# marcinmiklitz/pywindow

Hardware: AMD Instinct MI355X
Metric: trajectory frames/sec full_analysis (pore+windows), CC3 1k-frame (higher is better)
Workload: dtype f64

## Files before the change

### pywindow_amd/csrc/pw_unit.hpp

```cpp
#pragma once
#include "../../include/pywindow_amd.h"
#include "pw_lbfgsb.hpp"
#include "pw_math.hpp"
#include "pw_team.hpp"
#include <string.h>

#if defined(PW_PROFILE) && defined(__HIPCC__)
__shared__ unsigned long long pw_prof_lds[32];
#define PW_PROF_BASE(ws) ((unsigned long long*)pw_prof_lds)
#endif
#if defined(PW_PROFILE) && defined(__HIP_DEVICE_COMPILE__)
#define PW_T0(var) long long var = wall_clock64()
#if defined(PW_ZPROF) && defined(PW_LB_FINE)
#define PW_T1(ws, slot, var) do { (void)var; } while (0)
#elif defined(PW_BARRIER_PROF)
#define PW_T1(ws, slot, var) do { (void)var; if (T::lane() == 0) { unsigned long long w_ = 0; \
        for (int k_ = 0; k_ < T::NWAVES; ++k_) w_ += atomicExch(&pw_bar_acc[k_], 0ull); \
        atomicAdd(&pw_prof_lds[slot], w_); } } while (0)
#else
#define PW_T1(ws, slot, var) do { if (T::lane() == 0) atomicAdd(&pw_prof_lds[slot], (unsigned long long)(wall_clock64() - var)); } while (0)
#endif
#else
#define PW_T0(var) do {} while (0)
#define PW_T1(ws, slot, var) do {} while (0)
// ... 1131 lines not shown
    return ::asin(x);
#else
    return __builtin_asin(x);
#endif
}
PW_HD inline double cone_atan2(double y, double x) {
#if defined(__HIP_DEVICE_COMPILE__)
    return ::atan2(y, x);
#else
    return __builtin_atan2(y, x);
#endif
}
PW_HD inline ConeLattice cone_lattice_window(double rx, double ry, double rz, double rr, double thr, double R) {
    ConeLattice L;
    L.c = 0.0; L.w = 1.0; L.j = -1; L.first = 0; L.plen = 1;
    const double len = pw_sqrt(rr);
    const double ct = thr / (R * len) - 1e-12;
    if (!(ct > 0.0)) return L;
    const double sa = pw_sqrt(pw_max(1.0 - ct * ct, 0.0));
    const double rho = pw_sqrt(rx * rx + ry * ry) / len;
    if (!(rho > sa * (1.0 + 1e-6) + 1e-9)) return L;
    const double delta = cone_asin(sa / rho) * (1.0 + 1e-9) + 1e-9;
    const double w = delta / ONE_PI;
    int j = 0;
    while (j + 1 < ConeLatticeTable::N && pw_abs(CONE_LATTICE_TABLE.s[j]) > w) ++j;
    if (j + 1 >= ConeLatticeTable::N) return L;
    double c = (cone_atan2(ry, rx) - delta) / TWO_PI;
    c -= __builtin_floor(c);
    L.c = c < 1.0 ? c : 0.0;
    L.w = w;
    L.j = (short)j;
    return L;
}
struct ConeLatticeWalk {
    double t, w, a, b;
    int k, A, B;
    PW_HD void enter(const ConeLattice& L, int k0, int kend) {
        const int j = L.j, pos = j & 1 ? j + 1 : j, neg = j & 1 ? j : j + 1;
        A = CONE_LATTICE_TABLE.q[pos]; a = CONE_LATTICE_TABLE.s[pos];
        B = CONE_LATTICE_TABLE.q[neg]; b = -CONE_LATTICE_TABLE.s[neg];
        w = L.w;
        k = k0;
        t = (double)k0 * CONE_LATTICE_G - L.c;
        t -= __builtin_floor(t);
        while (k <= kend && !(t < w)) {
            ++k;
            t += CONE_LATTICE_G;
            if (t >= 1.0) t -= 1.0;
        }
    }
    PW_HD void next() {
        if (t + a < w) { k += A; t += a; }
        else if (t - b >= 0.0) { k += B; t -= b; }
        else { k += A + B; t = (t + a) - b; }
    }
};
PW_HD inline ConeLattice* take_cone_lattice(ScratchArena& a, int n) {
#ifdef PW_NO_CONE_LATTICE
    (void)a; (void)n;
    return nullptr;
#else
    return (ConeLattice*)a.take((size_t)(n + 1) * sizeof(ConeLattice));
#endif
}
PW_HD inline __attribute__((always_inline)) int cone_of_atom(double rx, double ry, double rz, double vr, double cn, const Sphere& sp,
                                                            bool narrow, ConeBand* out, ConeLattice* lat_out) {
    const int P = sp.P;
    ConeBand b;
    ConeLattice L;
    L.c = 0.0; L.w = 1.0; L.j = -1; L.first = 0; L.plen = 1;
    int cnt = 0;
    const double rr = sq3(rx, ry, rz);
    const double a2 = rr - pw_fma(rr, 1e-12, (vr * vr) * (1.0 + 1e-12));
    b.klo = 0; b.khi = -P;
    b.thr = -PW_INF;
    if (a2 > 0.0) {
        const double amin = pw_sqrt(a2) * (1.0 - 1e-9);
        b.thr = amin * sp.R * (1.0 - 1e-9);
        if (amin > cn + 1e-6) {
            const double len = pw_sqrt(rr);
            const double zd = rz / len, c = amin / len;
            const double s_ = pw_sqrt(pw_max(1.0 - c * c, 0.0)) * (1.0 + 1e-9) + 1e-9;
            const double rho = pw_sqrt(pw_max(1.0 - zd * zd, 0.0));
            const double zhi = zd >= c ? 1.0 : pw_min(1.0, zd * c + rho * s_ + 1e-9);
            const double zlo = zd <= -c ? -1.0 : pw_max(-1.0, zd * c - rho * s_ - 1e-9);
            const double kh = (zlo - sp.start) / sp.step, kl = (zhi - sp.start) / sp.step;
            b.klo = (int)pw_max(kl - 2.0, 0.0);
            b.khi = (int)pw_min(kh + 3.0, (double)(P - 1));
            if (narrow) {
                L = cone_lattice_window(rx, ry, rz, rr, b.thr, sp.R);
                if (L.j >= 0) {
                    cnt = cone_pieces(b.khi - b.klo + 1, L.w, &L.plen);
                    b.klo = ~b.klo;
                }
            }
        }
    }
    *out = b;
    *lat_out = L;
    return cnt;
}
template <class T, bool FAR, class GETP>
PW_HD inline __attribute__((always_inline)) bool team_ray_tests(const Frame& F, int n, const double* cen, const Sphere& sp,
                                                               GETP getp, ConeBand* bands, unsigned* pairs, int cap,
                                                               PW_LDS int* counts, unsigned char* flag,
                                                               unsigned char hit_value, double* far,
                                                               ConeLattice* lat = nullptr) {
    const int P = sp.P;
    const int seg = cap / T::NWAVES;
    if (P >= 65536 || n >= 65536 || seg < 64) return false;
    const double c0 = cen[0], c1 = cen[1], c2 = cen[2];
    const double cn = norm3(c0, c1, c2);
    int running = 0;
    for (int base = 0; base < n; base += T::SIZE) {
        const int i = base + T::tid();
        ConeBand b;
        ConeLattice L;
        int cnt = 0;
        if (i < n) {
            cnt = cone_of_atom(F.x[i] - c0, F.y[i] - c1, F.z[i] - c2, F.vdw[i], cn, sp, lat != nullptr, &b, &L);
            bands[i] = b;
        }
        if (lat != nullptr) {
            const int inc = T::incl_scan_i(cnt);
            if (T::lane() == T::WSIZE - 1) counts[T::wave()] = inc;
            T::sync();
            int at = running + inc - cnt;
#pragma unroll
            for (int w = 0; w < T::NWAVES; ++w) { const int cw = counts[w]; if (w < T::wave()) at += cw; running += cw; }
            if (i < n) { L.first = at; lat[i] = L; }
            T::sync();
        }
    }
    if (lat != nullptr && T::tid() == 0) lat[n].first = running;
    T::sync();
    int mine = 0;
    unsigned* my = pairs + (size_t)T::wave() * seg;
    auto enumerate = [&](auto bands_, auto lat_, auto my_) __attribute__((always_inline)) {
        for (int g0 = T::wave() * T::WSIZE; g0 < running; g0 += T::SIZE) {
            const int g = g0 + T::lane();
            ConeLatticeWalk wk;
            wk.k = 1;
            int kend = 0, i = 0;
            double rx = 0.0, ry = 0.0, rz = 0.0, thr = 0.0;
            if (g < running) {
                int lo = 0, hi = n - 1;
                while (lo < hi) {
                    const int mid = (lo + hi) >> 1;
                    if (lat_[mid + 1].first > g) hi = mid; else lo = mid + 1;
                }
                i = lo;
                const ConeBand b = bands_[i];
                const ConeLattice L = lat_[i];
                const int k0 = ~b.klo + (g - L.first) * (int)L.plen;
                kend = k0 + (int)L.plen - 1 < b.khi ? k0 + (int)L.plen - 1 : b.khi;
                rx = F.x[i] - c0; ry = F.y[i] - c1; rz = F.z[i] - c2;
                thr = b.thr;
                wk.enter(L, k0, kend);
            }
            while (T::wave_any(wk.k <= kend)) {
                const bool act = wk.k <= kend;
                const int k = wk.k;
                bool f = false;
                if (act) {
                    double px, py, pz;
                    getp(k, &px, &py, &pz);
                    const double dot = pw_fma(pz, rz, pw_fma(px, rx, py * ry));
                    f = dot >= thr;
                    wk.next();
                }
                const unsigned long long bal = T::ballot(f);
                const int pos = mine + __builtin_popcountll(bal & ((1ull << T::lane()) - 1ull));
                if (f && pos < seg) my_[pos] = ((unsigned)k << 16) | (unsigned)i;
                mine += __builtin_popcountll(bal);
            }
        }
    };
    if (lat != nullptr) {
        if (PW_IS_LDS(bands) && PW_IS_LDS(lat) && PW_IS_LDS(my)) enumerate(PW_AS_LDS(bands), PW_AS_LDS(lat), PW_AS_LDS(my));
        else enumerate(bands, lat, my);
    }
    for (int i = T::wave(); i < n; i += T::NWAVES) {
        const ConeBand b = bands[i];
        if (b.klo < 0) continue;
        const bool two_sided = b.khi < 0;
        const int khi = two_sided ? -b.khi - 1 : b.khi;
        const double rx = F.x[i] - c0, ry = F.y[i] - c1, rz = F.z[i] - c2;
        int off = getp.first(b.klo + T::lane());
        for (int kb = b.klo; kb <= khi; kb += T::WSIZE, off += GETP::STEP64) {
            const int k = kb + T::lane();
            bool f = false;
            if (k <= khi) {
                double px, py, pz;
                if (T::WSIZE == 64) getp.at(off, &px, &py, &pz);
                else getp(k, &px, &py, &pz);
                const double dot = pw_fma(pz, rz, pw_fma(px, rx, py * ry));
                f = two_sided ? pw_abs(dot) >= b.thr : dot >= b.thr;
            }
            const unsigned long long bal = T::ballot(f);
            const int pos = mine + __builtin_popcountll(bal & ((1ull << T::lane()) - 1ull));
            if (f && pos < seg) my[pos] = ((unsigned)k << 16) | (unsigned)i;
            mine += __builtin_popcountll(bal);
        }
    }
    if (T::lane() == 0) counts[T::wave()] = mine;
    T::sync();
    int cum[T::NWAVES + 1];
    cum[0] = 0;
    bool fits = true;
#pragma unroll
    for (int w = 0; w < T::NWAVES; ++w) { const int cw = counts[w]; fits = fits && cw <= seg; cum[w + 1] = cum[w] + cw; }
    T::sync();
    if (!fits) return false;
    for (int g = T::tid(); g < cum[T::NWAVES]; g += T::SIZE) {
        int w = 0, first = 0;
#pragma unroll
        for (int q = 1; q < T::NWAVES; ++q)
            if (g >= cum[q]) { w = q; first = cum[q]; }
        const unsigned pr = pairs[(size_t)w * seg + (g - first)];
        const int k = (int)(pr >> 16), i = (int)(pr & 0xffffu);
        double dx, dy, dz;
        getp(k, &dx, &dy, &dz);
        const double nrm = norm3(dx, dy, dz);
        const double ux = dx / nrm, uy = dy / nrm, uz = dz / nrm;
        const double rx = F.x[i] - c0, ry = F.y[i] - c1, rz = F.z[i] - c2;
        const double along = pw_fma(rz, uz, pw_fma(rx, ux, ry * uy));
        const double sq = sq3(rx, ry, rz);
        const double perp = pw_sqrt(sq - along * along);
        const double radicand = F.vdw[i] * F.vdw[i] - perp * perp;
        if (radicand > 0.0) {
            const double half = pw_sqrt(radicand);
            const double tin = along - half, tout = along + half;
            const double ix = c0 + tin * ux, iy = c1 + tin * uy, iz = c2 + tin * uz;
            const double ox = c0 + tout * ux, oy = c1 + tout * uy, oz = c2 + tout * uz;
            const double nin = norm3(ix, iy, iz), nout = norm3(ox, oy, oz);
            if (nin < nout) {
                flag[k] = hit_value;
                if (FAR) team_store_max_pos(&far[k], nout);
            }
        }
    }
    T::sync();
    return true;
}

PW_HD inline double np_floordiv(double a, double b) {
    double mod = __builtin_fmod(a, b);
    double div = (a - mod) / b;
    if (mod != 0.0) {
        if ((b < 0.0) != (mod < 0.0)) div -= 1.0;
    }
    double fl;
    if (div != 0.0) {
        fl = __builtin_floor(div);
        if (div - fl > 0.5) fl += 1.0;
    } else {
        fl = 0.0;
    }
    return fl;
}

PW_NOINLINE PW_HD inline bool path_scan_thread(const Frame& F, int n, double vx, double vy, double vz,
                                   double inc, double m0, double* out_2gap, int* out_pos, double* out_chunk,
                                   int* n_eval, const lint* cand = nullptr, const lint* coff = nullptr) {
    double nrm = norm3(vx, vy, vz);
    int chunks = (int)np_floordiv(nrm, inc);
    double cx = vx / (double)chunks, cy = vy / (double)chunks, cz = vz / (double)chunks;
    double best = PW_INF;
    int pos = 0;
    bool ok = true;
    int k0 = 0;
    if (chunks >= 1) {
        if (!(m0 > 0.0)) ok = false;
        best = m0;
        k0 = 1;
    }
    auto tile = [&](auto np_) __attribute__((always_inline)) {
        constexpr int NP = decltype(np_)::value;
        double qx[NP], qy[NP], qz[NP], m[NP];
#pragma unroll
        for (int p = 0; p < NP; ++p) {
            int k = k0 + p <= chunks ? k0 + p : chunks;
            qx[p] = cx * (double)k; qy[p] = cy * (double)k; qz[p] = cz * (double)k;
        }
        points_gap_values<NP>(F, n, qx, qy, qz, m, cand, coff);
#pragma unroll
        for (int p = 0; p < NP; ++p) {
            if (k0 + p <= chunks && ok) {
                if (!(m[p] > 0.0)) ok = false;
                else if (m[p] < best) { best = m[p]; pos = k0 + p; }
            }
        }
        k0 += NP;
    };
    while (k0 <= chunks && ok) {
        if (chunks - k0 + 1 <= 5) tile(std::integral_constant<int, 5>());
        else tile(std::integral_constant<int, 6>());
    }
    if (n_eval) *n_eval += chunks + 1;
    if (!ok) return false;
    *out_2gap = best * 2.0;
    *out_pos = pos;
    out_chunk[0] = cx; out_chunk[1] = cy; out_chunk[2] = cz;
    return true;
}

template <class T>
PW_HD inline bool wave_path_candidates(const Frame& F, int n, bool have, double vx, double vy, double vz, double inc,
                                       double m0, lint* cand, lint* coff) {
    const auto& C = *F.cls;
    if (C.k == 0 || !(m0 > 0.0)) return false;
    double uz_lo = PW_INF, uz_hi = -PW_INF, t1 = PW_INF;
    bool odd = false;
    if (have) {
        const double nrm = norm3(vx, vy, vz);
        odd = !(nrm >= inc * (1.0 + 1e-9)) || !(nrm < PW_INF) || !(inc > 0.0);
        if (!odd) uz_lo = uz_hi = vz / nrm;
    }
    if (T::wave_any(odd)) return false;
    double z1 = T::wave_min(uz_lo) - 1e-9, z2 = -T::wave_min(-uz_hi) + 1e-9;
    t1 = inc * (1.0 - 1e-9);
    if (!(z1 <= z2)) return false;
    z1 = pw_max(z1, -1.0); z2 = pw_min(z2, 1.0);
    const double s1 = pw_sqrt(pw_max(1.0 - z1 * z1, 0.0)), s2 = pw_sqrt(pw_max(1.0 - z2 * z2, 0.0));
    const double m0p = m0 * (1.0 + 1e-9) + 1e-9;
    const int mycut = T::lane() <= C.k ? C.off[T::lane() <= PW_KCLS ? T::lane() : PW_KCLS] : n;
    int mycount = 0, cnt = 0;
    for (int base = 0; base < n; base += T::WSIZE) {
        const int i = base + T::lane();
        bool keep = false;
        if (i < n) {
            const double xx = F.xx[i], z = F.z[i], r = F.vdw[i];
            const double rho = pw_sqrt(xx);
            const double zd = rho > 0.0 ? z / rho : 0.0;
            const double sd = pw_sqrt(pw_max(1.0 - zd * zd, 0.0));
            double c1 = 1.0;
            if (zd > z2) c1 = sd * s2 + zd * z2;
            else if (zd < z1) c1 = sd * s1 + zd * z1;
            c1 = pw_min(1.0, pw_max(0.0, c1 + 1e-9));
            const double ts = rho * c1;
            const double low = ts >= t1 ? xx * (1.0 - c1 * c1) : (xx + t1 * t1) - 2.0 * t1 * ts;
            const double lim = (r + m0p) * (r + m0p);
            keep = !(low * (1.0 - 1e-9) - 1e-9 > lim * (1.0 + 1e-9));
        }
        const unsigned long long bal = T::ballot(keep);
        const int pos = cnt + __builtin_popcountll(bal & ((1ull << T::lane()) - 1ull));
        if (keep) cand[pos] = i;
        if (T::WSIZE > 1) {
            int w = mycut - base;
            w = w < 0 ? 0 : (w > 64 ? 64 : w);
            mycount += __builtin_popcountll(bal & (w >= 64 ? ~0ull : ((1ull << w) - 1ull)));
        }
        cnt += __builtin_popcountll(bal);
    }
    if (T::WSIZE > 1) {
        if (T::lane() <= C.k) coff[T::lane()] = mycount;
    } else {
        int c = 0;
        for (int g = 0; g <= C.k; ++g) {
            while (c < cnt && cand[c] < C.off[g]) ++c;
            coff[g] = c;
        }
    }
    T::wave_sync();
    return true;
}

PW_HD inline size_t template_groups_bytes(int n) {
    const size_t npad = (size_t)((n + 1) & ~1);
    return ((sizeof(ClassInfo) + 7) & ~(size_t)7) + npad * 4 * 2 + npad * 8 + 8;
}
PW_HD inline double molecular_weight_sum(const double* mass, int n) {
    double tot = 0.0;
    for (int s0 = 0; s0 < n; s0 += 8192) {
        double part = np_sum_lean(mass + s0, n - s0 < 8192 ? n - s0 : 8192);
        tot = s0 == 0 ? part : tot + part;
    }
    return tot;
}
inline void template_groups_build(const double* vdw, const double* mass, int n, unsigned char* blob) {
    const size_t npad = (size_t)((n + 1) & ~1);
    ClassInfo* cls = (ClassInfo*)blob;
    int* inv = (int*)(blob + ((sizeof(ClassInfo) + 7) & ~(size_t)7));
    int* perm = inv + npad;
    double* vs = (double*)(perm + npad);
    memset(blob, 0, template_groups_bytes(n));
    int ngrp = 0;
    for (int i = 0; i < n; ++i) {
        int key = i;
        for (int j = 0; j < i; ++j)
            if (vdw[j] == vdw[i]) { key = j; break; }
        perm[i] = key;
        if (key == i) ++ngrp;
    }
    if (ngrp > PW_KCLS) {
        cls->k = 0; cls->off[0] = 0;
        for (int i = 0; i < n; ++i) inv[i] = i;
    } else {
        cls->k = ngrp;
        for (int i = 0; i < n; ++i) {
            const int key = perm[i];
            int pos = 0, cid = 0;
            for (int j = 0; j < n; ++j) {
                const int kj = perm[j];
                pos += (kj < key) || (kj == key && j < i);
                cid += (kj == j) && (j < key);
            }
            inv[i] = pos;
            if (key == i) { cls->vdw[cid] = vdw[i]; cls->off[cid] = pos; }
        }
        cls->off[ngrp] = n;
    }
    for (int i = 0; i < n; ++i) { vs[inv[i]] = vdw[i]; }
    for (int i = 0; i < n; ++i) perm[inv[i]] = i;
    vs[npad] = molecular_weight_sum(mass, n);
}

template <class T>
PW_HD inline void load_unit(UnitShared& sh, int n, const double* xyz, const double* vdw,
                            const double* mass, const unsigned char* tmpl = nullptr) {
    auto& v = *sh.v;
    if (tmpl) {
        const size_t npad = (size_t)((n + 1) & ~1);
        const ClassInfo* tc = (const ClassInfo*)tmpl;
        const int* t_inv = (const int*)(tmpl + ((sizeof(ClassInfo) + 7) & ~(size_t)7));
        const int* t_perm = t_inv + npad;
        const double* t_vs = (const double*)(t_perm + npad);
        for (int i = T::tid(); i < n; i += T::SIZE) {
            const int pos = t_inv[i];
            const double x = xyz[3 * i], y = xyz[3 * i + 1], z = xyz[3 * i + 2];
            sh.A.x[pos] = x; sh.A.y[pos] = y; sh.A.z[pos] = z;
            sh.A.xx[pos] = sq3(x, y, z);
            sh.inv[i] = pos;
            sh.perm[i] = t_perm[i];
            sh.vdw[i] = t_vs[i];
            sh.mass[i] = mass[i];
        }
        if (T::tid() == 0) {
            v.n_eval = 0; v.status = 0;
            v.mw = t_vs[npad]; v.mw_given = 1;
            v.cls.k = tc->k;
            for (int g = 0; g <= PW_KCLS; ++g) v.cls.off[g] = tc->off[g];
            for (int g = 0; g < PW_KCLS; ++g) v.cls.vdw[g] = tc->vdw[g];
        }
        T::sync();
        return;
    }
    for (int i = T::tid(); i < n; i += T::SIZE) {
        double r = vdw[i];
        sh.vdw[i] = r;
        sh.mass[i] = mass[i];
    }
    if (T::tid() == 0) { v.n_eval = 0; v.status = 0; v.cls.k = 0; v.mw_given = 0; }
    T::sync();
    for (int i = T::tid(); i < n; i += T::SIZE) {
        double r = sh.vdw[i];
        int key = i;
        for (int j = 0; j < i; ++j)
            if (sh.vdw[j] == r) { key = j; break; }
        sh.perm[i] = key;
    }
    T::sync();
    for (int i = T::tid(); i < n; i += T::SIZE) {
        int key = sh.perm[i];
        int pos = 0, cid = 0;
        for (int j = 0; j < n; ++j) {
            int kj = sh.perm[j];
            pos += (kj < key) || (kj == key && j < i);
            cid += (kj == j) && (j < key);
        }
        sh.inv[i] = pos;
        if (key == i) {
            if (cid < PW_KCLS) { v.cls.vdw[cid] = sh.vdw[i]; v.cls.off[cid] = pos; }
            team_atomic_max(&v.cls.k, cid + 1);
        }
    }
    T::sync();
    const int ngrp = v.cls.k;
    T::sync();
    if (ngrp > PW_KCLS) {
        for (int i = T::tid(); i < n; i += T::SIZE) sh.inv[i] = i;
        if (T::tid() == 0) { v.cls.k = 0; v.cls.off[0] = 0; }
    } else if (T::tid() == 0) {
        v.cls.off[ngrp] = n;
    }
    T::sync();
    for (int i = T::tid(); i < n; i += T::SIZE) {
        int pos = sh.inv[i];
        double x = xyz[3 * i], y = xyz[3 * i + 1], z = xyz[3 * i + 2];
        sh.A.x[pos] = x; sh.A.y[pos] = y; sh.A.z[pos] = z;
        sh.A.xx[pos] = sq3(x, y, z);
        sh.vdw[pos] = vdw[i];
        sh.perm[pos] = i;
    }
    T::sync();
}

template <int B, class F>
PW_HD inline double seq_sum_blocks(int n, F term) {
    double s = term(0);
    int i = 1;
    for (; i + B <= n; i += B) {
        double v[B];
#pragma unroll
        for (int j = 0; j < B; ++j) v[j] = term(i + j);
#pragma unroll
        for (int j = 0; j < B; ++j) s = s + v[j];
    }
    for (; i < n; ++i) s = s + term(i);
    return s;
}
template <class F>
PW_HD inline double seq_sum_blocked(int n, F term) { return seq_sum_blocks<8>(n, term); }

template <class T>
PW_HD inline ldouble* seq_sum_columns(const UnitShared& sh, int n) {
    const size_t np = (size_t)((n + 1) & ~1);
    if (T::SIZE < 64 || sh.scratch_bytes < 3 * np * 8) return nullptr;
    return (ldouble*)sh.scratch;
}
template <class T, class FIN>
PW_HD inline void seq_sum_columns_add(const ldouble* cols, int n, FIN fin) {
    const size_t np = (size_t)((n + 1) & ~1);
    if (T::tid() < 3) {
        const ldouble* a = cols + (size_t)T::tid() * np;
        fin(T::tid(), seq_sum_blocks<16>(n, [&](int i) { return a[i]; }));
    }
}

template <class T>
PW_HD inline void make_shifted(UnitShared& sh, int n, double cx, double cy, double cz) {
    ldouble* cols = seq_sum_columns<T>(sh, n);
    const size_t np = (size_t)((n + 1) & ~1);
    for (int i = T::tid(); i < n; i += T::SIZE) {
        double x = sh.A.x[i] - cx, y = sh.A.y[i] - cy, z = sh.A.z[i] - cz;
        sh.S.x[i] = x; sh.S.y[i] = y; sh.S.z[i] = z;
        sh.S.xx[i] = sq3(x, y, z);
        if (cols) { const int ci = sh.perm[i]; cols[ci] = x; cols[np + ci] = y; cols[2 * np + ci] = z; }
    }
    T::sync();
    if (cols) {
        seq_sum_columns_add<T>(cols, n, [&](int c, double s) { sh.v->centroid[c] = s / (double)n; });
        T::sync();
        return;
    }
    auto cen_comp = [&](int c) {
        const ldouble* a = c == 0 ? sh.S.x : (c == 1 ? sh.S.y : sh.S.z);
        double s = seq_sum_blocked(n, [&](int i) { return a[sh.inv[i]]; });
        sh.v->centroid[c] = s / (double)n;
    };
    if (T::SIZE >= 3) {
        if (T::tid() < 3) cen_comp(T::tid());
    } else if (T::tid() == 0) {
        cen_comp(0); cen_comp(1); cen_comp(2);
    }
    T::sync();
}

struct GramEdgeRule {
    int t0, panel, panel_wide, nfull, limlast;
    PW_HD static bool applies(int n) { return n % 8 >= 4; }
    PW_HD static int last_panel_start(int n) {
        int start = 0;
        for (;;) {
            const int rem = n - start;
            const int mi = rem >= 384 ? 192 : (rem > 192 ? 32 * ((rem / 2 + 31) / 32) : rem);
            if (start + mi >= n) return start;
            start += mi;
        }
    }
    PW_HD explicit GramEdgeRule(int n) {
        t0 = applies(n) ? 8 * (n / 8) : 0x40000000;
        panel = last_panel_start(n);
        panel_wide = 12 * (panel / 12);
        nfull = 32 * (n / 32);
        limlast = 12 * ((n - nfull) / 12);
    }
    PW_HD bool is_edge(int o) const { return (unsigned)(o - t0) < 4u; }
    PW_HD bool in_wide_kernel(int o) const {
        return o < panel ? o < panel_wide : (o & 31) < (o < nfull ? 24 : limlast);
    }
    PW_HD bool pair_uses_edge_order(int oi, int oj) const {
        return (is_edge(oi) && in_wide_kernel(oj)) || (is_edge(oj) && in_wide_kernel(oi));
    }
};
template <bool EDGE>
PW_HD inline __attribute__((always_inline)) double pw_gram_nn(double xi, double yi, double zi, double xj, double yj,
                                                              double zj, int oi, int oj, const GramEdgeRule& er) {
    if (EDGE && er.pair_uses_edge_order(oi, oj)) return pw_fma(zi, zj, xi * xj + yi * yj);
    return pw_fma(zi, zj, pw_fma(yi, yj, xi * xj));
}

#if defined(__HIP_DEVICE_COMPILE__)
template <class T, bool VALUE_ONLY, bool EDGE>
__device__ inline __attribute__((always_inline)) bool team_max_dim_few(UnitShared& sh, const Frame& F, int n,
                                                                       const GramEdgeRule& er, const double* centre) {
    auto& v = *sh.v;
    const double cx = centre ? centre[0] : 0.0, cy = centre ? centre[1] : 0.0, cz = centre ? centre[2] : 0.0;
    double smax = -PW_INF, nmax = 0.0;
    int imax = 0x7fffffff;
    for (int i = T::tid(); i < n; i += T::SIZE) {
        const double dx = F.x[i] - cx, dy = F.y[i] - cy, dz = F.z[i] - cz;
        const double si = pw_sqrt(dx * dx + dy * dy + dz * dz) + F.vdw[i];
        if (si > smax) { smax = si; imax = i; }
        nmax = pw_max(nmax, F.xx[i]);
    }
// ... 1509 lines not shown
            v.status |= PW_ST_PATH_TOO_LONG;
            out->n_points = 0; out->sphere_r = radius; out->n_windows = -1; out->n_clusters = 0; out->n_survivors = 0; out->eps = 0.0;
        }
        T::sync();
        return -1;
    }
    int P = sampling_count(radius, prm.adjust_windows);
    if (T::tid() == 0) {
        out->n_points = P;
        out->sphere_r = radius;
        out->n_windows = -1;
        out->n_clusters = 0;
        out->n_survivors = 0;
        out->eps = 0.0;
    }
    if (P > ws->p_cap || P < 10) {
        if (T::tid() == 0) v.status |= P < 10 ? PW_ST_TOO_FEW_POINTS : PW_ST_POINTS_OVERFLOW;
        T::sync();
        return -1;
    }
    Sphere sp;
    sp.init(radius, P);
    ScratchArena arena;
    arena.init(sh);
    const int Q4 = (P + 3) >> 2;
    double* pts = (double*)arena.take((size_t)Q4 * 12 * 8);
    if (!pts) pts = ws->pts;
    auto PT = [Q4](int k, int c) { return (c * 4 + (k & 3)) * Q4 + (k >> 2); };
    ScratchArena arena_pts = arena;
    team_sphere_points<T>(ws, sp, [&](int k, double x, double y, double z) { pts[PT(k, 0)] = x; pts[PT(k, 1)] = y; pts[PT(k, 2)] = z; });
    T::sync();
    if (T::wave() == 0) PW_T1(ws, 26, t_pre);
    PW_T0(t_eps);
    {
        PW_T0(t_knn);
        constexpr int NK = 4;
        const int ngroups = (P + NK - 1) / NK;
        int* s_tab = (int*)arena.take(324 * 4);
        double* s_leaf = (double*)arena.take(256 * 8);
        double* s_acc = nullptr;
        double* tile = nullptr;
        int tile_cap = 0;
        if (s_tab && s_leaf && T::SIZE > 1 && ngroups <= T::SIZE) {
            long words = (long)(arena.left / 8) - 160;
            int slots = (int)(words / (64 + 8)) - 2;
            if (slots > 64) slots = 64;
            if (slots >= 4) {
                size_t acc_words = 8 * (size_t)(slots + 2);
                if (acc_words < 128) acc_words = 128;
                s_acc = (double*)arena.take(acc_words * 8);
                tile = (double*)arena.take((size_t)slots * 64 * 8);
                tile_cap = slots * 64 - 128;
            }
        }
        const bool streamed = tile != nullptr && s_acc != nullptr && tile_cap >= 128;
        if (!streamed) {
            arena = arena_pts;
            s_tab = (int*)arena.take(324 * 4);
            s_acc = (double*)arena.take(8 * 160 * 8);
            s_leaf = (double*)arena.take(256 * 8);
            if (!s_tab || !s_acc || !s_leaf) { s_tab = ws->leaf_tab; s_acc = ws->acc8; s_leaf = ws->leaf; }
        }
        const unsigned short* nb_idx = nullptr;
        const double* nb_bound = nullptr;
        if (ws->nb_off && P >= PW_NB_PMIN && P <= PW_NB_PMAX && ws->nb_off[P] != PW_NB_NONE) {
            nb_idx = ws->nb_idx + (size_t)ws->nb_off[P] * PW_NB_K;
            nb_bound = ws->nb_bound + ws->nb_off[P];
        }
        const int W = (int)(0.118 * (double)P) + 6;
        const double zstep = pw_abs(sp.step) * radius;
        auto point_tabled = [&](auto pts_, int k, double* d10) __attribute__((always_inline)) {
            if (!nb_idx) return false;
            const double slack = (radius * radius) * (1.0 - 1e-9);
            const double px = pts_[PT(k, 0)], py = pts_[PT(k, 1)], pz = pts_[PT(k, 2)];
            const unsigned* row = (const unsigned*)(nb_idx + (size_t)k * PW_NB_K);
            unsigned w[8];
#pragma unroll
            for (int c = 0; c < 8; ++c) w[c] = row[c];
            double prev = -1.0, cd[PW_NB_K];
            bool sorted = true;
#pragma unroll
            for (int c = 0; c < PW_NB_K; ++c) {
                const int j = (int)((w[c >> 1] >> (16 * (c & 1))) & 0xffffu);
                const double qx = pts_[PT(j, 0)], qy = pts_[PT(j, 1)], qz = pts_[PT(j, 2)];
                double ax = px - qx, ay = py - qy, az = pz - qz;
                double d = ax * ax;
                d = d + ay * ay; d = d + az * az;
                sorted = sorted && d >= prev;
                prev = d;
                cd[c] = d;
                if (c < 10) d10[c] = d;
            }
            if (!sorted) {
#pragma unroll
                for (int q = 0; q < 10; ++q) d10[q] = PW_INF;
#pragma unroll
                for (int c = 0; c < PW_NB_K; ++c) {
                    double v_ = cd[c];
#pragma unroll
                    for (int q = 0; q < 10; ++q) {
                        double lo_ = __builtin_fmin(d10[q], v_);
                        v_ = __builtin_fmax(d10[q], v_);
                        d10[q] = lo_;
                    }
                }
            }
            const bool ok = d10[9] < nb_bound[k] * slack;
#pragma unroll
            for (int q = 0; q < 10; ++q) d10[q] = pw_sqrt(d10[q]);
            return ok;
        };
        auto point_dists = [&](auto pts_, int grp, int k, bool& searched, double* d10) __attribute__((always_inline)) {
            if (!searched && point_tabled(pts_, k, d10)) return;
            if (!searched) {
                knn_window_group(pts_, Q4, P, grp, W, radius, zstep, ws->knn);
                searched = true;
            }
#pragma unroll
            for (int q = 0; q < 10; ++q) d10[q] = ws->knn[(size_t)k * 10 + q];
        };
        if (!streamed) {
            auto rows_of_groups = [&](auto pts_) __attribute__((always_inline)) {
                for (int grp = T::tid(); grp < ngroups; grp += T::SIZE) {
                    bool searched = false;
                    for (int p = 0; p < NK; ++p) {
                        const int k = grp * NK + p;
                        if (k >= P) break;
                        double d10[10];
                        point_dists(pts_, grp, k, searched, d10);
                        if (!searched) {
#pragma unroll
                            for (int q = 0; q < 10; ++q) ws->knn[(size_t)k * 10 + q] = d10[q];
                        }
                    }
                }
            };
            if (PW_IS_LDS(pts)) rows_of_groups(PW_AS_LDS(pts)); else rows_of_groups(pts);
        }
        T::sync();
        if (T::wave() == 0) PW_T1(ws, 24, t_knn);
        PW_T0(t_sum);
        double sum;
        if (streamed) {
            const int n_el = P * 10;
            const int grp = T::tid();
            const int e_first = grp * NK * 10;
            bool searched = false;
            double total = 0.0;
            bool first = true;
            for (int s0 = 0; s0 < n_el; s0 += 8192) {
                const int len = n_el - s0 < 8192 ? n_el - s0 : 8192;
                np_leaf_table<T>(len, s_tab);
                int lo = 0;
                while (lo < len) {
                    int hi = len;
                    if (lo + tile_cap < len) {
                        int off, l;
                        np_descend(len, lo + tile_cap, &off, &l);
                        hi = off;
                    }
                    auto fill = [&](auto tile_, auto pts_) __attribute__((always_inline)) {
                        if (nb_idx) {
                            const int E0 = s0 + lo, E1 = s0 + hi;
                            const int k1 = (E1 - 1) / 10;
                            for (int k = E0 / 10 + T::tid(); k <= k1; k += T::SIZE) {
                                double d10[10];
                                if (!point_tabled(pts_, k, d10)) {
                                    knn_window_group(pts_, Q4, P, k / NK, W, radius, zstep, ws->knn);
#pragma unroll
                                    for (int q = 0; q < 10; ++q) d10[q] = ws->knn[(size_t)k * 10 + q];
                                }
                                const int e0 = k * 10 - s0;
#pragma unroll
                                for (int q = 0; q < 10; ++q)
                                    if (e0 + q >= lo && e0 + q < hi) tile_[e0 + q - lo] = d10[q];
                            }
                            return;
                        }
                        if (grp >= ngroups) return;
                        for (int p = 0; p < NK; ++p) {
                            const int k = grp * NK + p;
                            const int e0 = e_first + p * 10 - s0;
                            if (k >= P || e0 + 10 <= lo || e0 >= hi) continue;
                            double d10[10];
                            point_dists(pts_, grp, k, searched, d10);
#pragma unroll
                            for (int q = 0; q < 10; ++q)
                                if (e0 + q >= lo && e0 + q < hi) tile_[e0 + q - lo] = d10[q];
                        }
                    };
                    if (PW_IS_LDS(tile) && PW_IS_LDS(pts)) fill(PW_AS_LDS(tile), PW_AS_LDS(pts)); else fill(tile, pts);
                    T::sync();
                    np_leaf_phase<T>(tile, len, lo, hi, s_tab, s_acc, s_leaf, true);
                    lo = hi;
                }
                double part = np_walk_phase<T>(len, s_tab, s_acc, s_leaf);
                if (T::tid() == 0) total = first ? part : total + part;
                first = false;
                T::sync();
            }
            if (T::tid() == 0) v.red_v[15] = total;
            T::sync();
            sum = v.red_v[15];
            T::sync();
        } else {
            sum = np_sum_team<T>(ws->knn, P * 10, s_tab, s_acc, s_leaf, &v.red_v[15]);
        }
        double m = sum / (double)(P * 10);
        if (T::tid() == 0) { v.eps = m + pw_pow_np(m, 0.5); out->eps = v.eps; }
        T::sync();
        if (T::wave() == 0) PW_T1(ws, 25, t_sum);
    }
    if (T::wave() == 0) PW_T1(ws, 8, t_eps);
    PW_T0(t_smp);
    arena = arena_pts;
    double* vals = (double*)arena.take((size_t)P * 8);
    if (!vals) vals = ws->vals;
    int* surv_k = (int*)arena.take((size_t)P * 4);
    if (!surv_k) surv_k = ws->surv_k;
    int* labels = (int*)arena.take((size_t)P * 4);
    if (!labels) labels = ws->labels;
    unsigned char* flag = (unsigned char*)arena.take((size_t)P);
    if (!flag) flag = ws->flag;
    ScratchArena arena_mark = arena;
    double* tmpv = (double*)arena.take((size_t)P * 8);
    if (!tmpv) tmpv = ws->knn;
    {
        double cen[3] = {v.centroid[0], v.centroid[1], v.centroid[2]};
        bool done = false;
        {
            for (int k = T::tid(); k < P; k += T::SIZE) flag[k] = 1;
            ScratchArena a2 = arena_mark;
            ConeBand* bands = (ConeBand*)a2.take((size_t)n * sizeof(ConeBand));
            ConeLattice* lat = bands ? take_cone_lattice(a2, n) : nullptr;
            int cap = (int)(a2.left / 4);
            unsigned* pairs = (unsigned*)a2.take((size_t)cap * 4);
            if (cap < 4 * P) { pairs = (unsigned*)ws->knn; cap = 16 * ws->p_cap; }
            if (!bands && (size_t)n * sizeof(ConeBand) <= (size_t)ws->p_cap * 16) bands = (ConeBand*)(ws->knn + 8 * (size_t)ws->p_cap);
            auto run = [&](auto pts_) __attribute__((always_inline)) {
                SpiralRays<decltype(pts_)> getp{pts_, Q4};
                return team_ray_tests<T, false>(sh.S, n, cen, sp, getp, bands, pairs, cap, (PW_LDS int*)&v.red_i[0], flag, 0, nullptr, lat);
            };
            if (bands) done = PW_IS_LDS(pts) ? run(PW_AS_LDS(pts)) : run(pts);
        }
        if (done) {
        } else if (T::SIZE > 1) {
            constexpr int NR = 4;
            for (int k0 = T::tid(); k0 < P; k0 += NR * T::SIZE) {
                double dx[NR], dy[NR], dz[NR], far[NR];
                bool hit[NR];
#pragma unroll
                for (int r = 0; r < NR; ++r) {
                    int k = k0 + r * T::SIZE < P ? k0 + r * T::SIZE : k0;
                    dx[r] = pts[PT(k, 0)]; dy[r] = pts[PT(k, 1)]; dz[r] = pts[PT(k, 2)];
                }
                ray_scan_multi<NR, false>(sh.S, n, cen, dx, dy, dz, hit, far);
#pragma unroll
                for (int r = 0; r < NR; ++r) {
                    int k = k0 + r * T::SIZE;
                    if (k < P) flag[k] = hit[r] ? 0 : 1;
                }
            }
        } else {
            for (int k = T::tid(); k < P; k += T::SIZE) {
                double far;
                bool hit = ray_scan(sh.S, n, cen, pts[PT(k, 0)], pts[PT(k, 1)], pts[PT(k, 2)], &far);
                flag[k] = hit ? 0 : 1;
            }
        }
        T::sync();
        if (T::wave() == 0) {
            int m = 0;
            for (int base = 0; base < P; base += T::WSIZE) {
                int k = base + T::lane();
                bool f = k < P && flag[k] != 0;
                unsigned long long bal = T::ballot(f);
                int pos = m + __builtin_popcountll(bal & ((1ull << T::lane()) - 1ull));
                if (f) labels[pos] = k;
                m += __builtin_popcountll(bal);
            }
            if (T::lane() == 0) v.n_surv = m;
        }
        T::sync();
        int ncand = v.n_surv;
        int evals = 0;
        if (T::wave() == 0) PW_T1(ws, 30, t_smp);
        PW_T0(t_path);
        const double m_origin = wave_gap_value<T>(sh.S, n, 0.0, 0.0, 0.0);
        int whole = T::SIZE > 1 ? (ncand / T::SIZE) * T::SIZE : ncand;
        if ((ncand - whole) * 16 >= T::SIZE) whole = ncand;
        lint* cand_w = nullptr;
        lint* coff_w = nullptr;
        {
            ScratchArena a3 = arena;
            const size_t per_wave = (size_t)n + PW_KCLS + 2;
            int* c_all = (int*)a3.take((size_t)T::NWAVES * per_wave * 4);
#ifndef PW_NO_SCAN_LISTS
            if (c_all && PW_IS_LDS(c_all)) {
                cand_w = (lint*)PW_AS_LDS(c_all) + (size_t)T::wave() * per_wave;
                coff_w = cand_w + n;
            }
#endif
        }
        for (int j0 = 0; j0 < whole; j0 += T::SIZE) {
            const int j = j0 + T::tid();
            const bool have = j < whole;
            const int k = have ? labels[j] : 0;
            const double vx = pts[PT(k, 0)], vy = pts[PT(k, 1)], vz = pts[PT(k, 2)];
            const bool listed = cand_w != nullptr &&
                                wave_path_candidates<T>(sh.S, n, have, vx, vy, vz, prm.increment, m_origin, cand_w, coff_w);
            if (have) {
                double g2, chunk[3];
                int pos;
                bool ok = path_scan_thread(sh.S, n, vx, vy, vz, prm.increment, m_origin, &g2, &pos, chunk, &evals,
                                           listed ? cand_w : nullptr, listed ? coff_w : nullptr);
                flag[j] = ok ? 1 : 0;
                tmpv[j] = g2;
            }
        }
        const int left = ncand - whole;
        if (left > 0) {
            for (int j = whole + T::wave(); j < ncand; j += T::NWAVES) {
                const int k = labels[j];
                const double vx = pts[PT(k, 0)], vy = pts[PT(k, 1)], vz = pts[PT(k, 2)];
                const int chunks = (int)np_floordiv(norm3(vx, vy, vz), prm.increment);
                double g2 = 0.0;
                bool ok = true;
                bool all_at_once = false;
                if constexpr (T::WSIZE == 64) all_at_once = chunks >= 1 && chunks <= 16 && sh.S.cls->k > 0;
                if (all_at_once) {
                    if constexpr (T::WSIZE == 64) {
                        const auto& C = *sh.S.cls;
                        const Frame& F = sh.S;
                        const double cx = vx / (double)chunks, cy = vy / (double)chunks, cz = vz / (double)chunks;
                        const int sub = T::lane() & 3;
                        const int q = (T::lane() >> 2) + 1 <= chunks ? (T::lane() >> 2) + 1 : chunks;
                        const double qx = cx * (double)q, qy = cy * (double)q, qz = cz * (double)q;
                        const double pp = sq3(qx, qy, qz);
                        double gap = PW_INF;
                        for (int g = 0; g < C.k; ++g) {
                            double m2 = PW_INF;
                            const int hi = C.off[g + 1];
                            for (int i = C.off[g] + sub; i < hi; i += 4) {
                                const double x = F.x[i], y = F.y[i], z = F.z[i], xx = F.xx[i];
                                const double gg = pw_fma(z, qz, pw_fma(x, qx, y * qy));
                                m2 = __builtin_fmin(m2, pw_m2add(gg, xx));
                            }
                            m2 = __builtin_fmin(m2, T::xor_d(m2, 1));
                            m2 = __builtin_fmin(m2, T::xor_d(m2, 2));
                            const double m2p = m2 + pp;
                            const double d = pw_sqrt(m2p > 0.0 ? m2p : 0.0);
                            gap = __builtin_fmin(gap, d - C.vdw[g]);
                        }
                        double best = m_origin;
                        if (!(m_origin > 0.0)) ok = false;
                        for (int q2 = 1; q2 <= chunks && ok; ++q2) {
                            const double m = T::bcast_u(gap, 4 * (q2 - 1));
                            if (!(m > 0.0)) ok = false;
                            else if (m < best) best = m;
                        }
                        g2 = best * 2.0;
                    }
                } else if (chunks >= 1) {
                    const double cx = vx / (double)chunks, cy = vy / (double)chunks, cz = vz / (double)chunks;
                    double best = m_origin;
                    if (!(m_origin > 0.0)) ok = false;
                    for (int q = 1; q <= chunks && ok; ++q) {
                        const double m = wave_gap_value<T>(sh.S, n, cx * (double)q, cy * (double)q, cz * (double)q);
                        if (!(m > 0.0)) ok = false;
                        else if (m < best) best = m;
                    }
                    g2 = best * 2.0;
                } else {
                    double chunk[3];
                    int pos;
                    ok = path_scan_thread(sh.S, n, vx, vy, vz, prm.increment, m_origin, &g2, &pos, chunk, &evals);
                }
                if (T::lane() == 0) { flag[j] = ok ? 1 : 0; tmpv[j] = g2; }
            }
        }
        T::sync();
        if (T::wave() == 0) PW_T1(ws, 31, t_path);
        if (T::wave() == 0) {
            int m = 0;
            for (int base = 0; base < ncand; base += T::WSIZE) {
                int j = base + T::lane();
                bool f = j < ncand && flag[j] != 0;
                unsigned long long bal = T::ballot(f);
                int pos = m + __builtin_popcountll(bal & ((1ull << T::lane()) - 1ull));
                if (f) { surv_k[pos] = labels[j]; vals[pos] = tmpv[j]; }
                m += __builtin_popcountll(bal);
            }
            if (T::lane() == 0) { v.n_surv = m; out->n_survivors = m; }
        }
        T::sync();
        (void)evals;
    }
    if (T::wave() == 0) PW_T1(ws, 9, t_smp);
    int ns = v.n_surv;
    if (ns == 0) {
        if (T::tid() == 0) out->n_windows = -1;
        T::sync();
        return -1;
    }
    PW_T0(t_db);
    arena = arena_mark;
    {
        const int label = team_dbscan<T>(sh.bits[0], sh.bits[1], sh.bits[2], arena, ws, pts, PT, surv_k, ns, v.eps, labels);
        if (label < 0) {
            if (T::tid() == 0) v.status |= PW_ST_POINTS_OVERFLOW;
            T::sync();
            return -1;
        }
        if (T::tid() == 0) {
            v.n_clusters = label;
            out->n_clusters = label;
        }
        if (label > PW_W_MAX) {
            wa.vec = ws->xw; wa.d = ws->xw + 3 * (size_t)ws->p_cap; wa.c = ws->xw + 4 * (size_t)ws->p_cap; wa.ok = ws->xw_ok;
        }
        for (int c = T::tid(); c < label; c += T::SIZE) wa.ok[c] = 0;
        T::sync();
        for (int c = T::wave(); c < label; c += T::NWAVES) {
            double best = -PW_INF;
            int bidx = 0x7fffffff;
            for (int q = T::lane(); q < ns; q += T::WSIZE) {
                if (labels[q] == c) {
                    double val = vals[q];
                    if (val > best || (val == best && q < bidx)) { best = val; bidx = q; }
                }
            }
            T::wave_argmax(best, bidx);
            if (T::lane() == 0) {
                const int pvk = surv_k[bidx];
                wa.vec[3 * c] = pts[PT(pvk, 0)]; wa.vec[3 * c + 1] = pts[PT(pvk, 1)]; wa.vec[3 * c + 2] = pts[PT(pvk, 2)];
            }
        }
        T::sync();
        if (pw_unit_debug* dbg = ws->dbg_base ? ws->dbg_base + ws->unit : nullptr) {
            for (int i = T::tid(); i < ns && i < PW_P_MAX; i += T::SIZE) {
                dbg->pass_idx[i] = surv_k[i];
                dbg->labels[i] = labels[i];
                dbg->gap2[i] = vals[i];
            }
            if (T::tid() == 0) { dbg->n_survivors = ns; dbg->n_clusters = label; }
        }
    }
    if (T::wave() == 0) PW_T1(ws, 10, t_db);
    return v.n_clusters;
}

PW_HD inline int windows_finish(const WinArrays& wa, int ncl, pw_unit_out* out, TeamWorkspace* ws, long unit) {
    int st = 0, m = 0;
    for (int c = 0; c < ncl; ++c) {
        if (wa.ok[c] > 0) {
            const double wd = wa.d[c];
            if (m < PW_W_MAX) {
                out->win_d[m] = wd;
                out->win_c[m][0] = wa.c[3 * c];
                out->win_c[m][1] = wa.c[3 * c + 1];
                out->win_c[m][2] = wa.c[3 * c + 2];
            } else {
                st |= PW_ST_WINDOW_OVERFLOW;
                unsigned slot = team_atomic_inc(ws->xwin_count);
                if (ws->xwin && slot < ws->xwin_cap) {
                    pw_extra_window* e = ws->xwin + slot;
                    e->unit = unit; e->index = m; e->reserved = 0; e->d = wd;
                    e->c[0] = wa.c[3 * c]; e->c[1] = wa.c[3 * c + 1]; e->c[2] = wa.c[3 * c + 2];
                }
            }
            if (wd < 0.0) st |= PW_ST_WINDOW_NEGATIVE;
            ++m;
        } else if (wa.ok[c] < 0) {
            st |= PW_ST_Z_BOUNDS;
        } else {
            st |= PW_ST_WINDOW_DROPPED;
        }
    }
    out->n_windows = m;
    return st;
}

template <class T>
PW_HD inline __attribute__((always_inline)) void stage_windows_impl(UnitShared& sh, TeamWorkspace* ws, int n, pw_unit_out* out,
                                                                    const pw_params& prm) {
    auto& v = *sh.v;
    WinArrays wa;
    wa.vec = (double*)&v.win_vec[0][0]; wa.d = (double*)v.win_d; wa.c = (double*)&v.win_c[0][0]; wa.ok = (int*)v.win_ok;
    if (windows_bulk_impl<T>(sh, ws, n, out, prm, wa) < 0) return;
    PW_T0(t_w);
    const int ncl = v.n_clusters;
    int nslot = T::NWAVES < 4 ? T::NWAVES : 4;
    if (sh.nslots < nslot) nslot = sh.nslots;
    if (T::wave() < nslot) {
        const double shift[3] = {v.shift[0], v.shift[1], v.shift[2]};
        for (int c = T::wave(); c < ncl; c += nslot)
            wave_window<T>(sh.S, sh.R[T::wave()], sh.lb[T::wave()], ws, n, c, shift, prm, wa, (int*)&v.red_i[8 + T::wave()]);
    }
    T::sync();
    if (T::wave() == 0) PW_T1(ws, 12, t_w);
    if (T::tid() == 0) {
        v.status |= windows_finish(wa, ncl, out, ws, ws->unit);
        for (int w = 0; w < T::NWAVES && w < 8; ++w) v.n_eval += v.red_i[8 + w];
    }
    T::sync();
}

template <class T>
PW_NOINLINE PW_HD inline void stage_windows(UnitShared& sh, TeamWorkspace* ws, int n, pw_unit_out* out,
                                             const pw_params& prm) {
    stage_windows_impl<T>(sh, ws, n, out, prm);
}

constexpr unsigned PW_STAGE_REUSE_OPT = 16u;
constexpr unsigned PW_STAGE_MERGE = 32u;
constexpr unsigned PW_STAGE_COM_ONLY = 64u;

PW_HD inline void record_or_status(pw_unit_out* out, int st, int evals) {
#if defined(__HIP_DEVICE_COMPILE__)
    if (st) atomicOr(&out->status, st);
    atomicAdd(&out->n_eval, evals);
#else
    out->status |= st;
    out->n_eval += evals;
#endif
}

template <class T>
PW_HD inline void analyse_unit(UnitShared& sh, TeamWorkspace* ws, int n, const double* xyz,
                               const double* vdw, const double* mass, unsigned stages,
                               pw_unit_out* out, const pw_params& prm, const unsigned char* tmpl = nullptr) {
    const bool merge = (stages & PW_STAGE_MERGE) != 0;
    const bool reuse_opt = (stages & PW_STAGE_REUSE_OPT) != 0;
    if ((stages & PW_STAGE_WINDOWS) && !reuse_opt && prm.pore_opt) stages |= PW_STAGE_OPT;
    if (T::tid() == 0 && !merge) {
        out->status = 0;
        out->n_eval = 0;
        out->avg_d = 0.0;
        out->pore_opt_d = 0.0; out->pore_opt_atom = -1; out->pore_vol_opt = 0.0;
        out->pore_opt_c[0] = out->pore_opt_c[1] = out->pore_opt_c[2] = 0.0;
        out->n_windows = -1; out->n_clusters = 0;
        out->n_points = 0; out->n_points_avg = 0; out->n_survivors = 0;
        out->opt_nit = 0; out->opt_nfev = 0; out->opt_task = 0; out->opt_msg = 0;
        out->eps = 0.0; out->sphere_r = 0.0;
        for (int w = 0; w < PW_W_MAX; ++w) {
            out->win_d[w] = 0.0;
            out->win_c[w][0] = out->win_c[w][1] = out->win_c[w][2] = 0.0;
        }
    }
    PW_T0(t_load);
    load_unit<T>(sh, n, xyz, vdw, mass, tmpl);
    if (T::wave() == 0) PW_T1(ws, 5, t_load);
    if (reuse_opt) {
        if (T::tid() == 0) { sh.v->com[0] = out->com[0]; sh.v->com[1] = out->com[1]; sh.v->com[2] = out->com[2]; }
        T::sync();
    } else {
        stage_basic<T>(sh, ws, n, out, (stages & PW_STAGE_COM_ONLY) != 0);
    }
    if (stages & PW_STAGE_OPT) stage_opt<T>(sh, ws, n, out, prm);
    if (reuse_opt) {
        if (T::tid() == 0) {
            sh.v->opt_c[0] = out->pore_opt_c[0];
            sh.v->opt_c[1] = out->pore_opt_c[1];
            sh.v->opt_c[2] = out->pore_opt_c[2];
            if (out->status & PW_ST_NEGATIVE_PORE) sh.v->status |= PW_ST_NEGATIVE_PORE;
        }
        T::sync();
    }
    if (stages & PW_STAGE_AVG) {
        PW_T0(t_a);
        stage_average<T>(sh, ws, n, out, prm);
        if (T::wave() == 0) PW_T1(ws, 13, t_a);
        if ((stages & PW_STAGE_WINDOWS) && sh.S.x == sh.A.x) {
            for (int i = T::tid(); i < n; i += T::SIZE) {
                const int pos = sh.inv[i];
                const double x = xyz[3 * i], y = xyz[3 * i + 1], z = xyz[3 * i + 2];
                sh.A.x[pos] = x; sh.A.y[pos] = y; sh.A.z[pos] = z;
                sh.A.xx[pos] = sq3(x, y, z);
            }
            T::sync();
        }
    }
    if (stages & PW_STAGE_WINDOWS) {
        if (!(prm.pore_opt && (sh.v->status & PW_ST_NEGATIVE_PORE))) {
            stage_windows<T>(sh, ws, n, out, prm);
        }
        else if (T::tid() == 0) out->n_windows = -1;
    }
    if (T::tid() == 0) {
        if (merge) {
            record_or_status(out, sh.v->status, sh.v->n_eval);
        } else {
            out->status = sh.v->status;
            out->n_eval = sh.v->n_eval;
        }
    }
    T::sync();
}

}
```

Measured before the change: 1.011 million.

## Bracket path minimum per atom analytically instead of scanning all chunks

Adds a path-scan variant that, for each atom, projects onto the path direction and evaluates only the two bracketing chunk points. This replaces a scan over every chunk along the path with constant work per atom. A numerical-safety bound based on the maximum squared norm decides per wave whether the bracket path is safe, and the code falls back to the full scan otherwise. It adds a wave reduction for xx_max and a second code path, and it changes what is computed, for example by not reporting the minimizing chunk position.

```diff
diff --git a/pywindow_amd/csrc/pw_unit.hpp b/pywindow_amd/csrc/pw_unit.hpp
--- a/pywindow_amd/csrc/pw_unit.hpp
+++ b/pywindow_amd/csrc/pw_unit.hpp
@@ -1457,6 +1457,77 @@
     *out_2gap = best * 2.0;
     *out_pos = pos;
     out_chunk[0] = cx; out_chunk[1] = cy; out_chunk[2] = cz;
+    return true;
+}
+
+struct PathSteps {
+    double cx, cy, cz, cd, rinv;
+    int chunks;
+    bool bracket;
+};
+PW_HD inline PathSteps path_steps(const Frame& F, double vx, double vy, double vz, double inc, double xx_max) {
+    PathSteps s;
+    const double nrm = norm3(vx, vy, vz);
+    const double fd = np_floordiv(nrm, inc);
+    s.bracket = F.cls->k > 0 && fd >= 1.0 && fd <= PW_PATH_POINTS_MAX && nrm < PW_INF;
+    s.chunks = s.bracket ? (int)fd : 0;
+    s.cd = (double)s.chunks;
+    s.cx = vx / s.cd; s.cy = vy / s.cd; s.cz = vz / s.cd;
+    const double cc = sq3(s.cx, s.cy, s.cz);
+    s.rinv = 1.0 / cc;
+    const double bound = (64.0 * 0x1p-53) * (xx_max + sq3(vx, vy, vz));
+    s.bracket = s.bracket && cc > 0.0 && cc < PW_INF && s.rinv < PW_INF && bound < PW_INF && cc * (1.0 - 1e-6) > bound;
+    return s;
+}
+PW_NOINLINE PW_HD inline bool path_bracket_thread(const Frame& F, int n, double cx, double cy, double cz, int chunks,
+                                                  double rinv, double m0, double* out_2gap, int* n_eval,
+                                                  const lint* cand = nullptr, const lint* coff = nullptr,
+                                                  long* n_terms = nullptr) {
+    (void)n;
+    const auto& C = *F.cls;
+    const double cd = (double)chunks;
+    double best = PW_INF;
+    long terms = 0;
+    for (int g = 0; g < C.k; ++g) {
+        double m2 = PW_INF;
+        auto atom = [&](double x, double y, double z, double xx) __attribute__((always_inline)) {
+            const double t = pw_fma(z, cz, pw_fma(x, cx, y * cy)) * rinv;
+            const double lo = __builtin_fmin(__builtin_fmax(__builtin_floor(t), 1.0), cd);
+            const double hi = __builtin_fmin(lo + 1.0, cd);
+            const double ax = cx * lo, ay = cy * lo, az = cz * lo;
+            const double bx = cx * hi, by = cy * hi, bz = cz * hi;
+            const double ga = pw_fma(z, az, pw_fma(x, ax, y * ay));
+            const double gb = pw_fma(z, bz, pw_fma(x, bx, y * by));
+            const double va = pw_m2add(ga, xx) + sq3(ax, ay, az);
+            const double vb = pw_m2add(gb, xx) + sq3(bx, by, bz);
+            m2 = __builtin_fmin(m2, __builtin_fmin(va, vb));
+        };
+        auto span = [&](int c, const int chi, auto at) __attribute__((always_inline)) {
+            terms += 2 * (chi - c);
+            for (; c + 4 <= chi; c += 4) {
+                int i[4];
+                double x[4], y[4], z[4], xx[4];
+#pragma unroll
+                for (int j = 0; j < 4; ++j) i[j] = at(c + j);
+#pragma unroll
+                for (int j = 0; j < 4; ++j) { x[j] = F.x[i[j]]; y[j] = F.y[i[j]]; z[j] = F.z[i[j]]; xx[j] = F.xx[i[j]]; }
+#pragma unroll
+                for (int j = 0; j < 4; ++j) atom(x[j], y[j], z[j], xx[j]);
+            }
+            for (; c < chi; ++c) {
+                const int i = at(c);
+                atom(F.x[i], F.y[i], F.z[i], F.xx[i]);
+            }
+        };
+        if (cand) span(coff[g], coff[g + 1], [&](int c) __attribute__((always_inline)) { return (int)cand[c]; });
+        else span(C.off[g], C.off[g + 1], [](int c) __attribute__((always_inline)) { return c; });
+        const double d = pw_sqrt(m2 > 0.0 ? m2 : 0.0);
+        best = __builtin_fmin(best, d - C.vdw[g]);
+    }
+    if (n_eval) *n_eval += chunks + 1;
+    if (n_terms) *n_terms += terms;
+    if (!(m0 > 0.0) || !(best > 0.0)) return false;
+    *out_2gap = (best < m0 ? best : m0) * 2.0;
     return true;
 }
 
@@ -3572,6 +3643,13 @@
             }
 #endif
         }
+#ifndef PW_NO_PATH_BRACKETS
+        double xx_max = 0.0;
+        if (whole > 0) {
+            for (int i = T::lane(); i < n; i += T::WSIZE) xx_max = __builtin_fmax(xx_max, sh.S.xx[i]);
+            xx_max = -T::wave_min(-xx_max);
+        }
+#endif
         for (int j0 = 0; j0 < whole; j0 += T::SIZE) {
             const int j = j0 + T::tid();
             const bool have = j < whole;
@@ -3579,6 +3657,19 @@
             const double vx = pts[PT(k, 0)], vy = pts[PT(k, 1)], vz = pts[PT(k, 2)];
             const bool listed = cand_w != nullptr &&
                                 wave_path_candidates<T>(sh.S, n, have, vx, vy, vz, prm.increment, m_origin, cand_w, coff_w);
+#ifndef PW_NO_PATH_BRACKETS
+            const PathSteps steps = path_steps(sh.S, vx, vy, vz, prm.increment, xx_max);
+            if (!T::wave_any(have && !steps.bracket)) {
+                if (have) {
+                    double g2 = 0.0;
+                    bool ok = path_bracket_thread(sh.S, n, steps.cx, steps.cy, steps.cz, steps.chunks, steps.rinv, m_origin,
+                                                  &g2, &evals, listed ? cand_w : nullptr, listed ? coff_w : nullptr);
+                    flag[j] = ok ? 1 : 0;
+                    tmpv[j] = g2;
+                }
+                continue;
+            }
+#endif
             if (have) {
                 double g2, chunk[3];
                 int pos;
```

New measurement: 1.041 million, median of 6. 1.03x the previous value.
